# codebits1001/CET-driven-simulation-for-3D-printing-AM-KMC-Approach

Hardware: NVIDIA B200
Metric: kmc_site_updates_per_s (higher is better)
Workload: dtype f64

## Files before the change

cet-driven-simulation-for-3d-printing-am-kmc-approach_b200/csrc/rates_refresh.cu:

```cuda
#include <algorithm>
#include "ctx.cuh"
#include "pair_walk.cuh"
#include "tile_state.cuh"

namespace cet {

int rate_tables_ensure(cet_ctx *c);
int sm_count(cet_ctx *c);

constexpr int RF_THREADS = 256, RF_WARPS = RF_THREADS / 32;
enum { RF_KM_EMPTY = 1u << 8, RF_KP_EMPTY = 1u << 9, RF_K_GT0 = 1u << 10, RF_K_LTL = 1u << 11 };

template <int ROWS>
struct RefreshSmem {
    static constexpr int RF_CHUNK = RF_WARPS * ROWS * 32;
    double op[RF_WARPS][14][32];
    double tab[RT_TABLE_DOUBLES];
    uint64_t lw[RF_CHUNK];
    int32_t ls[RF_CHUNK];
    uint32_t lc[RF_CHUNK];
    int n_list[2][2];
    unsigned int chunk[2];
};

struct RefreshArgs {
    const uint8_t *cvox;
    const double *pairop, *T;
    double *site_rate, *dep_rate;
    const double *tab;
    const int32_t *list;
    const unsigned int *n_list;
    unsigned int *queue;
    cet_rate_params P;
    int L, n0, i_off;
    int top_lo, top_hi;
    unsigned int mLL, mL;
    int lin[14];
};

__device__ __forceinline__ int fast_div(int n, int d, unsigned int m, int *rem)
{
    int q = (int)__umulhi((unsigned int)n, m);
    int r = n - q * d;
    if (r < 0) { --q; r += d; }
    *rem = r;
    return q;
}
__device__ __forceinline__ void cp_async8(uint32_t dst, const void *src)
{
    asm volatile("cp.async.ca.shared.global [%0], [%1], 8;" ::"r"(dst), "l"(src) : "memory");
}
__device__ __forceinline__ void cp_async_wait_all()
{
    asm volatile("cp.async.commit_group;\ncp.async.wait_group 0;" ::: "memory");
}

template <bool ATT>
__device__ __noinline__ double rf_pairs_slow(const cet_rate_params &P, const double *tab, int cnt, uint32_t opaddr, double A, double B, double sum)
{
    for (int r = 0; r < cnt; ++r) {
        const double op = lds_f64(opaddr + 256u * (uint32_t)r);
        sum += ATT ? att_pair_rate_E(P, op, A, B, tab) : diff_pair_rate(P, A, B, op);
    }
    return sum;
}
template <bool ATT>
__device__ __forceinline__ double rf_pairs(const cet_rate_params &P, const double *exp_tab, int cnt, uint32_t opaddr, double A, double B,
                                           const double sum0)
{
    double sum = sum0;
    int xmax = 0;
    uint32_t addr = opaddr;
    for (int r = 0; r < cnt; r += 2, addr += 512u) {
        const bool two = r + 1 < cnt;
        const double op0 = lds_f64(addr);
        double op1 = 0.0;
        if (two) op1 = lds_f64(addr + 256u);
        const double r0 = pair_rate_raw<ATT>(P, exp_tab, op0, A, B, xmax);
        const double r1 = pair_rate_raw<ATT>(P, exp_tab, op1, A, B, xmax);
        add_kept(P, sum, r0);
        if (two) add_kept(P, sum, r1);
    }
    if (ATT && xmax >= EXP_RANGE_HI) sum = rf_pairs_slow<ATT>(P, exp_tab, cnt, opaddr, A, B, sum0);
    return sum;
}

template <int ROWS>
__global__ void __launch_bounds__(RF_THREADS, 4) rates_refresh_kernel(const __grid_constant__ RefreshArgs a)
{
    constexpr int RF_CHUNK = RF_WARPS * ROWS * 32, RF_ROWS = ROWS;
    extern __shared__ __align__(16) unsigned char refresh_dyn_smem[];
    RefreshSmem<ROWS> &sm = *reinterpret_cast<RefreshSmem<ROWS> *>(refresh_dyn_smem);
    const cet_rate_params &P = a.P;
    const int tid = threadIdx.x, lane = tid & 31, wid = tid >> 5;
    const int L = a.L, LL = L * L;
    const unsigned lt_mask = (1u << lane) - 1u;
    const int n = (int)*a.n_list;

    for (int q = tid; q < RT_TABLE_DOUBLES; q += RF_THREADS) sm.tab[q] = a.tab[q];
    if (tid == 0) {
        sm.chunk[0] = atomicAdd(a.queue, 1u);
        sm.n_list[0][0] = 0; sm.n_list[0][1] = 0;
    }
    __syncthreads();
    const uint32_t op0 = (uint32_t)__cvta_generic_to_shared(&sm.op[wid][0][lane]);

    for (unsigned it = 0;; ++it) {
        const int64_t c0 = (int64_t)sm.chunk[it & 1u] * RF_CHUNK;
        if (c0 >= n) break;
        int *n_list = sm.n_list[it & 1u];
        if (tid == 0) {
            sm.chunk[(it + 1u) & 1u] = atomicAdd(a.queue, 1u);
            sm.n_list[(it + 1u) & 1u][0] = 0; sm.n_list[(it + 1u) & 1u][1] = 0;
        }
        const int hi = (int)(c0 + RF_CHUNK < n ? c0 + RF_CHUNK : n);

#pragma unroll
        for (int r = 0; r < RF_ROWS; ++r) {
            const int q = (int)c0 + 32 * (wid * RF_ROWS + r) + lane;
            const bool active = q < hi;
            const int s = active ? a.list[q] : 0;
            int rem, k;
            const int p = fast_div(s, LL, a.mLL, &rem), j = fast_div(rem, L, a.mL, &k);
            const int gi = a.i_off + p;
            const bool interior = (unsigned)(gi - 2) < (unsigned)(a.n0 - 4) && (unsigned)(j - 2) < (unsigned)(L - 4) &&
                                  (unsigned)(k - 2) < (unsigned)(L - 4);
            unsigned inb = 0x3FFFu;
            if (!__all_sync(0xffffffffu, interior || !active)) inb = inbounds_mask(gi, j, k, a.n0, L);
            const uint8_t *cs = a.cvox + s;
            unsigned c = 0, b[14], km = 0, kp = 0;
#pragma unroll
            for (int o = 0; o < 14; ++o) b[o] = 0;
            if (active) {
                c = cs[0];
                if (k > 0) km = cs[-1];
                if (k < L - 1) kp = cs[1];
#pragma unroll
                for (int o = 0; o < 14; ++o)
                    if (inb >> o & 1u) b[o] = cs[a.lin[o]];
            }
            uint32_t wlo = 0, whi = 0;
#pragma unroll
            for (int o = 0; o < 8; ++o) wlo += (b[o] & 15u) << (4 * o);
#pragma unroll
            for (int o = 8; o < 14; ++o) whi += (b[o] & 15u) << (4 * (o - 8));
            const unsigned code = c & 15u;
            const bool is_emp = active && code == TC_EMPTY;
            const bool is_occ = active && (code & 1u) && code != TC_DEFECT;
            const uint32_t emp = (~wlo & (wlo >> 3) & 0x11111111u) | (~whi & (whi >> 3) & 0x00111111u);
            const bool to_att = is_emp, to_diff = is_occ && emp != 0u;
            if (active && !to_att && !to_diff) {
                a.site_rate[s] = 0.0;
                if (s >= a.top_lo && s < a.top_hi) a.dep_rate[s - a.top_lo] = NAN;
            }
            const unsigned b_att = __ballot_sync(0xffffffffu, to_att), b_diff = __ballot_sync(0xffffffffu, to_diff);
            if (b_att | b_diff) {
                int base_a = 0, base_d = 0;
                if (lane == 0) {
                    if (b_att) base_a = atomicAdd(&n_list[0], __popc(b_att));
                    if (b_diff) base_d = atomicAdd(&n_list[1], __popc(b_diff));
                }
                base_a = __shfl_sync(0xffffffffu, base_a, 0); base_d = __shfl_sync(0xffffffffu, base_d, 0);
                const uint32_t ent = c | ((km & 15u) == TC_EMPTY ? RF_KM_EMPTY : 0u) | ((kp & 15u) == TC_EMPTY ? RF_KP_EMPTY : 0u) |
                                     (k > 0 ? RF_K_GT0 : 0u) | (k < L - 1 ? RF_K_LTL : 0u);
                const uint64_t w = (uint64_t)wlo | ((uint64_t)whi << 32);
                int pos = -1;
                if (to_att) pos = base_a + __popc(b_att & lt_mask);
                if (to_diff) pos = RF_CHUNK - 1 - base_d - __popc(b_diff & lt_mask);
                if (pos >= 0) { sm.lw[pos] = w; sm.ls[pos] = s; sm.lc[pos] = ent; }
            }
        }
        __syncthreads();

        const int n_att = n_list[0], n_diff = n_list[1];
        const int nb_att = (n_att + 31) >> 5, nb_all = nb_att + ((n_diff + 31) >> 5);
#pragma unroll 1
        for (int bt = wid; bt < nb_all; bt += RF_WARPS) {
            const bool att = bt < nb_att;
            const int q = att ? 32 * bt + lane : 32 * (bt - nb_att) + lane;
            const bool on = q < (att ? n_att : n_diff);
            const int pos = att ? q : RF_CHUNK - 1 - q;
            uint64_t w = 0;
            uint32_t e = 0;
            int s = 0;
            if (on) { w = sm.lw[pos]; s = sm.ls[pos]; e = sm.lc[pos]; }
            const uint64_t pm = !on ? 0ull : att ? (w & (w >> 3) & CET_NIB_LSB) : (~w & (w >> 3) & CET_NIB_LSB);
            const uint32_t pm_lo = (uint32_t)pm, pm_hi = (uint32_t)(pm >> 32);
            const int cnt = __popc(pm_lo) + __popc(pm_hi);
            {
                const double *src = a.pairop + s;
                uint32_t dst = op0;
#pragma unroll
                for (int o = 0; o < 14; ++o) {
                    if ((o < 8 ? pm_lo >> (4 * o) : pm_hi >> (4 * (o - 8))) & 1u) {
                        cp_async8(dst, src + a.lin[o]);
                        dst += 256u;
                    }
                }
            }
            if (att) {
                double T_self = 1.0, T_m = 1.0, T_p = 1.0;
                if (on) {
                    T_self = a.pairop[s];
                    T_m = T_self; T_p = T_self;
                    if (pm) {
                        if (e & RF_K_GT0) T_m = (e & RF_KM_EMPTY) ? a.pairop[s - 1] : a.T[s - 1];
                        if (e & RF_K_LTL) T_p = (e & RF_KP_EMPTY) ? a.pairop[s + 1] : a.T[s + 1];
                    }
                }
                const TilePrep pr = tile_prep_emp(P, sm.tab, w, T_self, T_m, T_p);
                cp_async_wait_all();
                if (on) {
                    a.site_rate[s] = cnt ? rf_pairs<true>(P, sm.tab + RT_EXP2, cnt, op0, pr.A, pr.B, pr.sum0) : pr.sum0;
                    if (s >= a.top_lo && s < a.top_hi) {
                        double dep;
                        a.dep_rate[s - a.top_lo] = dep_rate(P, T_self, &dep) ? dep : NAN;
                    }
                }
            } else {
                const double T_self = on ? a.T[s] : 1.0;
                const unsigned c = e & 255u;
                const TilePrep pr = tile_prep_occ(P, sm.tab, w, c & 15u, (int)(c >> 4), T_self);
                cp_async_wait_all();
                if (on) {
                    a.site_rate[s] = rf_pairs<false>(P, sm.tab + RT_EXP2, cnt, op0, pr.A, pr.B, 0.0);
                    if (s >= a.top_lo && s < a.top_hi) a.dep_rate[s - a.top_lo] = NAN;
                }
            }
        }
        __syncthreads();
    }
}

template <int ROWS>
static int refresh_launch(cet_ctx *c, const RefreshArgs &a, int64_t nsite_hint, int *blocks_per_sm)
{
    constexpr int CHUNK = RF_WARPS * ROWS * 32;
    const size_t smem = sizeof(RefreshSmem<ROWS>);
    if (*blocks_per_sm == 0) {
        CET_CUDA(cudaFuncSetAttribute(rates_refresh_kernel<ROWS>, cudaFuncAttributeMaxDynamicSharedMemorySize, (int)smem));
        int nb = 0;
        CET_CUDA(cudaOccupancyMaxActiveBlocksPerMultiprocessor(&nb, rates_refresh_kernel<ROWS>, RF_THREADS, smem));
        CET_REQUIRE(nb >= 1, "rates_refresh_kernel does not fit an SM");
        *blocks_per_sm = nb;
    }
    const int grid = (int)std::min<int64_t>((nsite_hint + CHUNK - 1) / CHUNK, (int64_t)sm_count(c) * *blocks_per_sm);
    rates_refresh_kernel<ROWS><<<grid, RF_THREADS, smem, c->stream>>>(a);
    CET_CUDA(cudaGetLastError());
    return 0;
}

int rates_refresh_list(cet_ctx *c, const int32_t *list, const unsigned int *counter, int64_t nsite_hint)
{
    if (int rc = rate_tables_ensure(c)) return rc;
    RefreshArgs a;
    memset(&a, 0, sizeof(a));
    a.cvox = c->cvox; a.pairop = c->pairop; a.T = c->T;
    a.site_rate = c->site_rate; a.dep_rate = c->dep_rate; a.tab = c->rate_tab;
    a.list = list; a.n_list = counter;
    a.queue = (unsigned int *)(c->rate_tab + RT_TABLE_DOUBLES) + 3;
    a.P = c->rp;
    a.L = (int)c->n1; a.n0 = (int)c->n0; a.i_off = (int)(c->i_begin - c->halo);
    const int64_t top = c->n0 - 1 - (c->i_begin - c->halo);
    if (top >= 0 && top < c->np) { a.top_lo = (int)(top * c->plane); a.top_hi = (int)((top + 1) * c->plane); }
    a.mLL = (unsigned int)((1ull << 32) / (uint64_t)c->plane) + 1u;
    a.mL = (unsigned int)((1ull << 32) / (uint64_t)c->n1) + 1u;
    for (int o = 0; o < 14; ++o) a.lin[o] = (h_nb_off[o][0] * a.L + h_nb_off[o][1]) * a.L + h_nb_off[o][2];
    CET_CUDA(cudaMemsetAsync(a.queue, 0, sizeof(unsigned int), c->stream));
    const int v = (c->debug_flags & 1048576) ? 0 : (c->debug_flags & 2097152) ? 2 : 1;
    if (v == 0) return refresh_launch<1>(c, a, nsite_hint, &c->refresh_blocks[0]);
    if (v == 2) return refresh_launch<4>(c, a, nsite_hint, &c->refresh_blocks[2]);
    return refresh_launch<2>(c, a, nsite_hint, &c->refresh_blocks[1]);
}

}
```

Baseline: 99.30 billion.

## Pipeline rate refresh: classify next chunk while computing current, sort by neighbor-count key

Restructures the refresh kernel so each thread classifies one site of the next chunk while the block computes rates for the current chunk. cp.async prefetch of pair operands and temperatures is issued during the classify phase rather than inside the compute loop. Listed sites are bucketed by class and pair count with match_any and a warp scan, so each warp handles sites with similar loop trip counts and less divergence. Results are staged in shared memory and written back coalesced by the owning thread. The cost is more shared memory, extra syncs per chunk, and a more complex chunk queue with two chunks in flight.

```diff
diff --git a/cet-driven-simulation-for-3d-printing-am-kmc-approach_b200/csrc/rates_refresh.cu b/cet-driven-simulation-for-3d-printing-am-kmc-approach_b200/csrc/rates_refresh.cu
--- a/cet-driven-simulation-for-3d-printing-am-kmc-approach_b200/csrc/rates_refresh.cu
+++ b/cet-driven-simulation-for-3d-printing-am-kmc-approach_b200/csrc/rates_refresh.cu
@@ -8,18 +8,21 @@
 int rate_tables_ensure(cet_ctx *c);
 int sm_count(cet_ctx *c);
 
-constexpr int RF_THREADS = 256, RF_WARPS = RF_THREADS / 32;
-enum { RF_KM_EMPTY = 1u << 8, RF_KP_EMPTY = 1u << 9, RF_K_GT0 = 1u << 10, RF_K_LTL = 1u << 11 };
-
-template <int ROWS>
+enum : uint32_t {
+    RF_KM_EMPTY = 1u << 8, RF_KP_EMPTY = 1u << 9, RF_K_GT0 = 1u << 10, RF_K_LTL = 1u << 11,
+    RF_LISTED = 1u << 12, RF_TOP = 1u << 13, RF_KEY_SHIFT = 14, RF_RANK_SHIFT = 19
+};
+constexpr uint64_t RF_CODES = 0x00FFFFFFFFFFFFFFull;
+
+template <int THREADS>
 struct RefreshSmem {
-    static constexpr int RF_CHUNK = RF_WARPS * ROWS * 32;
-    double op[RF_WARPS][14][32];
+    static constexpr int CHUNK = THREADS;
+    double op[14][CHUNK];
+    double sT[3][CHUNK];
+    uint64_t sw[CHUNK];
     double tab[RT_TABLE_DOUBLES];
-    uint64_t lw[RF_CHUNK];
-    int32_t ls[RF_CHUNK];
-    uint32_t lc[RF_CHUNK];
-    int n_list[2][2];
+    int key_cnt[2][32], key_start[2][32];
+    int n_cls[2][2];
     unsigned int chunk[2];
 };
 
@@ -55,197 +58,250 @@
     asm volatile("cp.async.commit_group;\ncp.async.wait_group 0;" ::: "memory");
 }
 
-template <bool ATT>
+template <bool ATT, uint32_t STRIDE>
 __device__ __noinline__ double rf_pairs_slow(const cet_rate_params &P, const double *tab, int cnt, uint32_t opaddr, double A, double B, double sum)
 {
     for (int r = 0; r < cnt; ++r) {
-        const double op = lds_f64(opaddr + 256u * (uint32_t)r);
+        const double op = lds_f64(opaddr + STRIDE * (uint32_t)r);
         sum += ATT ? att_pair_rate_E(P, op, A, B, tab) : diff_pair_rate(P, A, B, op);
     }
     return sum;
 }
-template <bool ATT>
+template <bool ATT, uint32_t STRIDE>
 __device__ __forceinline__ double rf_pairs(const cet_rate_params &P, const double *exp_tab, int cnt, uint32_t opaddr, double A, double B,
                                            const double sum0)
 {
     double sum = sum0;
     int xmax = 0;
     uint32_t addr = opaddr;
-    for (int r = 0; r < cnt; r += 2, addr += 512u) {
+    for (int r = 0; r < cnt; r += 2, addr += 2u * STRIDE) {
         const bool two = r + 1 < cnt;
         const double op0 = lds_f64(addr);
         double op1 = 0.0;
-        if (two) op1 = lds_f64(addr + 256u);
+        if (two) op1 = lds_f64(addr + STRIDE);
         const double r0 = pair_rate_raw<ATT>(P, exp_tab, op0, A, B, xmax);
         const double r1 = pair_rate_raw<ATT>(P, exp_tab, op1, A, B, xmax);
         add_kept(P, sum, r0);
         if (two) add_kept(P, sum, r1);
     }
-    if (ATT && xmax >= EXP_RANGE_HI) sum = rf_pairs_slow<ATT>(P, exp_tab, cnt, opaddr, A, B, sum0);
+    if (ATT && xmax >= EXP_RANGE_HI) sum = rf_pairs_slow<ATT, STRIDE>(P, exp_tab, cnt, opaddr, A, B, sum0);
     return sum;
 }
 
-template <int ROWS>
-__global__ void __launch_bounds__(RF_THREADS, 4) rates_refresh_kernel(const __grid_constant__ RefreshArgs a)
-{
-    constexpr int RF_CHUNK = RF_WARPS * ROWS * 32, RF_ROWS = ROWS;
+template <int THREADS>
+__global__ void __launch_bounds__(THREADS, 1024 / THREADS) rates_refresh_kernel(const __grid_constant__ RefreshArgs a)
+{
+    using Smem = RefreshSmem<THREADS>;
+    constexpr int CHUNK = Smem::CHUNK, WARPS = THREADS / 32;
+    constexpr uint32_t STRIDE = 8u * CHUNK;
     extern __shared__ __align__(16) unsigned char refresh_dyn_smem[];
-    RefreshSmem<ROWS> &sm = *reinterpret_cast<RefreshSmem<ROWS> *>(refresh_dyn_smem);
+    Smem &sm = *reinterpret_cast<Smem *>(refresh_dyn_smem);
     const cet_rate_params &P = a.P;
     const int tid = threadIdx.x, lane = tid & 31, wid = tid >> 5;
     const int L = a.L, LL = L * L;
     const unsigned lt_mask = (1u << lane) - 1u;
     const int n = (int)*a.n_list;
-
-    for (int q = tid; q < RT_TABLE_DOUBLES; q += RF_THREADS) sm.tab[q] = a.tab[q];
-    if (tid == 0) {
-        sm.chunk[0] = atomicAdd(a.queue, 1u);
-        sm.n_list[0][0] = 0; sm.n_list[0][1] = 0;
-    }
+    const uint32_t op0 = (uint32_t)__cvta_generic_to_shared(&sm.op[0][0]);
+    const uint32_t sT0 = (uint32_t)__cvta_generic_to_shared(&sm.sT[0][0]);
+    const unsigned past_end = (unsigned)(n / CHUNK + 1);
+    auto chunk_start = [&](unsigned e) { return (int)min(e, past_end) * CHUNK; };
+
+    auto classify = [&](int s_in, int b, uint64_t &w, uint32_t &lc) {
+        const bool active = s_in >= 0;
+        const int s = active ? s_in : 0;
+        int rem, k;
+        const int p = fast_div(s, LL, a.mLL, &rem), j = fast_div(rem, L, a.mL, &k);
+        const int gi = a.i_off + p;
+        const bool interior = (unsigned)(gi - 2) < (unsigned)(a.n0 - 4) && (unsigned)(j - 2) < (unsigned)(L - 4) &&
+                              (unsigned)(k - 2) < (unsigned)(L - 4);
+        unsigned inb = 0x3FFFu;
+        if (!__all_sync(0xffffffffu, interior || !active)) inb = inbounds_mask(gi, j, k, a.n0, L);
+        const uint8_t *cs = a.cvox + s;
+        unsigned c = 0, bc[14], km = 0, kp = 0;
+#pragma unroll
+        for (int o = 0; o < 14; ++o) bc[o] = 0;
+        if (active) {
+            c = cs[0];
+            if (k > 0) km = cs[-1];
+            if (k < L - 1) kp = cs[1];
+#pragma unroll
+            for (int o = 0; o < 14; ++o)
+                if (inb >> o & 1u) bc[o] = cs[a.lin[o]];
+        }
+        uint32_t wlo = 0, whi = 0;
+#pragma unroll
+        for (int o = 0; o < 8; ++o) wlo += (bc[o] & 15u) << (4 * o);
+#pragma unroll
+        for (int o = 8; o < 14; ++o) whi += (bc[o] & 15u) << (4 * (o - 8));
+        const unsigned code = c & 15u;
+        const bool is_emp = active && code == TC_EMPTY;
+        const bool is_occ = active && (code & 1u) && code != TC_DEFECT;
+        const uint32_t att = (wlo & (wlo >> 3) & 0x11111111u) | (whi & (whi >> 3) & 0x00111111u);
+        const uint32_t emp = (~wlo & (wlo >> 3) & 0x11111111u) | (~whi & (whi >> 3) & 0x00111111u);
+        const bool to_att = is_emp, to_diff = is_occ && emp != 0u;
+        const bool listed = to_att || to_diff;
+        const int key = (to_att ? 0 : 16) + __popc(to_att ? att : emp);
+        const unsigned peers = __match_any_sync(0xffffffffu, listed ? key : -1);
+        int rank = 0;
+        if (listed) {
+            const int leader = __ffs(peers) - 1;
+            if (lane == leader) rank = atomicAdd(&sm.key_cnt[b][key], __popc(peers));
+            rank = __shfl_sync(peers, rank, leader) + __popc(peers & lt_mask);
+        }
+        lc = (active && s >= a.top_lo && s < a.top_hi) ? RF_TOP : 0u;
+        if (listed)
+            lc |= c | ((km & 15u) == TC_EMPTY ? RF_KM_EMPTY : 0u) | ((kp & 15u) == TC_EMPTY ? RF_KP_EMPTY : 0u) | (k > 0 ? RF_K_GT0 : 0u) |
+                  (k < L - 1 ? RF_K_LTL : 0u) | RF_LISTED | ((uint32_t)key << RF_KEY_SHIFT) | ((uint32_t)rank << RF_RANK_SHIFT);
+        w = (uint64_t)wlo | ((uint64_t)whi << 32);
+    };
+    auto scan_keys = [&](int b) {
+        const int cnt = sm.key_cnt[b][lane];
+        int inc = cnt;
+#pragma unroll
+        for (int d = 1; d < 32; d <<= 1) {
+            const int u = __shfl_up_sync(0xffffffffu, inc, d);
+            if (lane >= d) inc += u;
+        }
+        const int n_emp = __shfl_sync(0xffffffffu, inc, 15);
+        sm.key_start[b][lane] = inc - cnt - (lane >= 16 ? n_emp : 0);
+        sm.key_cnt[b][lane] = 0;
+        if (lane == 31) { sm.n_cls[b][0] = n_emp; sm.n_cls[b][1] = inc - n_emp; }
+    };
+    auto sorted_pos = [&](uint32_t lc, int b) {
+        const int key = (int)((lc >> RF_KEY_SHIFT) & 31u);
+        const int i = sm.key_start[b][key] + (int)(lc >> RF_RANK_SHIFT);
+        return key < 16 ? i : CHUNK - 1 - i;
+    };
+
+    for (int q = tid; q < RT_TABLE_DOUBLES; q += THREADS) sm.tab[q] = a.tab[q];
+    if (tid < 64) sm.key_cnt[tid >> 5][tid & 31] = 0;
+    if (tid == 0) { sm.chunk[0] = atomicAdd(a.queue, 1u); sm.chunk[1] = atomicAdd(a.queue, 1u); }
     __syncthreads();
-    const uint32_t op0 = (uint32_t)__cvta_generic_to_shared(&sm.op[wid][0][lane]);
-
-    for (unsigned it = 0;; ++it) {
-        const int64_t c0 = (int64_t)sm.chunk[it & 1u] * RF_CHUNK;
-        if (c0 >= n) break;
-        int *n_list = sm.n_list[it & 1u];
-        if (tid == 0) {
-            sm.chunk[(it + 1u) & 1u] = atomicAdd(a.queue, 1u);
-            sm.n_list[(it + 1u) & 1u][0] = 0; sm.n_list[(it + 1u) & 1u][1] = 0;
-        }
-        const int hi = (int)(c0 + RF_CHUNK < n ? c0 + RF_CHUNK : n);
-
-#pragma unroll
-        for (int r = 0; r < RF_ROWS; ++r) {
-            const int q = (int)c0 + 32 * (wid * RF_ROWS + r) + lane;
-            const bool active = q < hi;
-            const int s = active ? a.list[q] : 0;
-            int rem, k;
-            const int p = fast_div(s, LL, a.mLL, &rem), j = fast_div(rem, L, a.mL, &k);
-            const int gi = a.i_off + p;
-            const bool interior = (unsigned)(gi - 2) < (unsigned)(a.n0 - 4) && (unsigned)(j - 2) < (unsigned)(L - 4) &&
-                                  (unsigned)(k - 2) < (unsigned)(L - 4);
-            unsigned inb = 0x3FFFu;
-            if (!__all_sync(0xffffffffu, interior || !active)) inb = inbounds_mask(gi, j, k, a.n0, L);
-            const uint8_t *cs = a.cvox + s;
-            unsigned c = 0, b[14], km = 0, kp = 0;
-#pragma unroll
-            for (int o = 0; o < 14; ++o) b[o] = 0;
-            if (active) {
-                c = cs[0];
-                if (k > 0) km = cs[-1];
-                if (k < L - 1) kp = cs[1];
-#pragma unroll
-                for (int o = 0; o < 14; ++o)
-                    if (inb >> o & 1u) b[o] = cs[a.lin[o]];
+    int c_cur = chunk_start(sm.chunk[0]);
+    int s_cur = c_cur + tid < n ? a.list[c_cur + tid] : -1, s_nxt = -1, s_pre;
+    uint64_t w_cur = 0, w_nxt = 0;
+    uint32_t lc_cur = 0, lc_nxt = 0;
+    if (c_cur < n) classify(s_cur, 0, w_cur, lc_cur);
+    {
+        const int c = chunk_start(sm.chunk[1]);
+        s_pre = c + tid < n ? a.list[c + tid] : -1;
+    }
+    __syncthreads();
+    if (wid == 0) scan_keys(0);
+    __syncthreads();
+
+    for (unsigned it = 0; c_cur < n; ++it) {
+        const int cur = it & 1u, nxt = cur ^ 1;
+        const int c_nxt = chunk_start(sm.chunk[nxt]);
+
+        if (lc_cur & RF_LISTED) {
+            const int pos = sorted_pos(lc_cur, cur);
+            const bool att = ((lc_cur >> RF_KEY_SHIFT) & 31u) < 16u;
+            const uint64_t w = w_cur, pm = att ? (w & (w >> 3) & CET_NIB_LSB) : (~w & (w >> 3) & CET_NIB_LSB);
+            const int s = s_cur;
+            const uint32_t pm_lo = (uint32_t)pm, pm_hi = (uint32_t)(pm >> 32);
+            const double *src = a.pairop + s;
+            uint32_t dst = op0 + 8u * (uint32_t)pos;
+#pragma unroll
+            for (int o = 0; o < 14; ++o) {
+                if ((o < 8 ? pm_lo >> (4 * o) : pm_hi >> (4 * (o - 8))) & 1u) {
+                    cp_async8(dst, src + a.lin[o]);
+                    dst += STRIDE;
+                }
             }
-            uint32_t wlo = 0, whi = 0;
-#pragma unroll
-            for (int o = 0; o < 8; ++o) wlo += (b[o] & 15u) << (4 * o);
-#pragma unroll
-            for (int o = 8; o < 14; ++o) whi += (b[o] & 15u) << (4 * (o - 8));
-            const unsigned code = c & 15u;
-            const bool is_emp = active && code == TC_EMPTY;
-            const bool is_occ = active && (code & 1u) && code != TC_DEFECT;
-            const uint32_t emp = (~wlo & (wlo >> 3) & 0x11111111u) | (~whi & (whi >> 3) & 0x00111111u);
-            const bool to_att = is_emp, to_diff = is_occ && emp != 0u;
-            if (active && !to_att && !to_diff) {
-                a.site_rate[s] = 0.0;
-                if (s >= a.top_lo && s < a.top_hi) a.dep_rate[s - a.top_lo] = NAN;
+            const uint32_t tdst = sT0 + 8u * (uint32_t)pos;
+            uint64_t fl;
+            if (att) {
+                cp_async8(tdst, a.pairop + s);
+                if (pm) {
+                    if (lc_cur & RF_K_GT0) cp_async8(tdst + STRIDE, ((lc_cur & RF_KM_EMPTY) ? a.pairop : a.T) + (s - 1));
+                    if (lc_cur & RF_K_LTL) cp_async8(tdst + 2u * STRIDE, ((lc_cur & RF_KP_EMPTY) ? a.pairop : a.T) + (s + 1));
+                }
+                fl = ((lc_cur >> 10) & 3u) | ((lc_cur & RF_TOP) ? 4u : 0u);
+            } else {
+                cp_async8(tdst, a.T + s);
+                fl = lc_cur & 255u;
             }
-            const unsigned b_att = __ballot_sync(0xffffffffu, to_att), b_diff = __ballot_sync(0xffffffffu, to_diff);
-            if (b_att | b_diff) {
-                int base_a = 0, base_d = 0;
-                if (lane == 0) {
-                    if (b_att) base_a = atomicAdd(&n_list[0], __popc(b_att));
-                    if (b_diff) base_d = atomicAdd(&n_list[1], __popc(b_diff));
-                }
-                base_a = __shfl_sync(0xffffffffu, base_a, 0); base_d = __shfl_sync(0xffffffffu, base_d, 0);
-                const uint32_t ent = c | ((km & 15u) == TC_EMPTY ? RF_KM_EMPTY : 0u) | ((kp & 15u) == TC_EMPTY ? RF_KP_EMPTY : 0u) |
-                                     (k > 0 ? RF_K_GT0 : 0u) | (k < L - 1 ? RF_K_LTL : 0u);
-                const uint64_t w = (uint64_t)wlo | ((uint64_t)whi << 32);
-                int pos = -1;
-                if (to_att) pos = base_a + __popc(b_att & lt_mask);
-                if (to_diff) pos = RF_CHUNK - 1 - base_d - __popc(b_diff & lt_mask);
-                if (pos >= 0) { sm.lw[pos] = w; sm.ls[pos] = s; sm.lc[pos] = ent; }
-            }
-        }
+            sm.sw[pos] = w | (fl << 56);
+        }
+        if (c_nxt < n) {
+            s_nxt = s_pre;
+            classify(s_nxt, nxt, w_nxt, lc_nxt);
+        }
+        cp_async_wait_all();
         __syncthreads();
-
-        const int n_att = n_list[0], n_diff = n_list[1];
+        if (tid == 0) sm.chunk[cur] = atomicAdd(a.queue, 1u);
+        if (wid == 0 && c_nxt < n) scan_keys(nxt);
+
+        const int n_att = sm.n_cls[cur][0], n_diff = sm.n_cls[cur][1];
         const int nb_att = (n_att + 31) >> 5, nb_all = nb_att + ((n_diff + 31) >> 5);
 #pragma unroll 1
-        for (int bt = wid; bt < nb_all; bt += RF_WARPS) {
+        for (int bt = wid; bt < nb_all; bt += WARPS) {
             const bool att = bt < nb_att;
             const int q = att ? 32 * bt + lane : 32 * (bt - nb_att) + lane;
             const bool on = q < (att ? n_att : n_diff);
-            const int pos = att ? q : RF_CHUNK - 1 - q;
+            const int pos = att ? q : CHUNK - 1 - q;
             uint64_t w = 0;
-            uint32_t e = 0;
-            int s = 0;
-            if (on) { w = sm.lw[pos]; s = sm.ls[pos]; e = sm.lc[pos]; }
-            const uint64_t pm = !on ? 0ull : att ? (w & (w >> 3) & CET_NIB_LSB) : (~w & (w >> 3) & CET_NIB_LSB);
-            const uint32_t pm_lo = (uint32_t)pm, pm_hi = (uint32_t)(pm >> 32);
-            const int cnt = __popc(pm_lo) + __popc(pm_hi);
-            {
-                const double *src = a.pairop + s;
-                uint32_t dst = op0;
-#pragma unroll
-                for (int o = 0; o < 14; ++o) {
-                    if ((o < 8 ? pm_lo >> (4 * o) : pm_hi >> (4 * (o - 8))) & 1u) {
-                        cp_async8(dst, src + a.lin[o]);
-                        dst += 256u;
-                    }
-                }
-            }
+            double T_self = 1.0;
+            if (on) { w = sm.sw[pos]; T_self = sm.sT[0][pos]; }
+            const unsigned fl = (unsigned)(w >> 56);
+            w &= RF_CODES;
+            const uint32_t opaddr = op0 + 8u * (uint32_t)pos;
             if (att) {
-                double T_self = 1.0, T_m = 1.0, T_p = 1.0;
-                if (on) {
-                    T_self = a.pairop[s];
-                    T_m = T_self; T_p = T_self;
-                    if (pm) {
-                        if (e & RF_K_GT0) T_m = (e & RF_KM_EMPTY) ? a.pairop[s - 1] : a.T[s - 1];
-                        if (e & RF_K_LTL) T_p = (e & RF_KP_EMPTY) ? a.pairop[s + 1] : a.T[s + 1];
-                    }
+                const uint64_t pm = w & (w >> 3) & CET_NIB_LSB;
+                double T_m = T_self, T_p = T_self;
+                if (pm) {
+                    if (fl & 1u) T_m = sm.sT[1][pos];
+                    if (fl & 2u) T_p = sm.sT[2][pos];
                 }
                 const TilePrep pr = tile_prep_emp(P, sm.tab, w, T_self, T_m, T_p);
-                cp_async_wait_all();
+                const int cnt = popc64(pm);
                 if (on) {
-                    a.site_rate[s] = cnt ? rf_pairs<true>(P, sm.tab + RT_EXP2, cnt, op0, pr.A, pr.B, pr.sum0) : pr.sum0;
-                    if (s >= a.top_lo && s < a.top_hi) {
+                    sm.sT[0][pos] = cnt ? rf_pairs<true, STRIDE>(P, sm.tab + RT_EXP2, cnt, opaddr, pr.A, pr.B, pr.sum0) : pr.sum0;
+                    if (fl & 4u) {
                         double dep;
-                        a.dep_rate[s - a.top_lo] = dep_rate(P, T_self, &dep) ? dep : NAN;
+                        sm.sT[1][pos] = dep_rate(P, T_self, &dep) ? dep : NAN;
                     }
                 }
             } else {
-                const double T_self = on ? a.T[s] : 1.0;
-                const unsigned c = e & 255u;
-                const TilePrep pr = tile_prep_occ(P, sm.tab, w, c & 15u, (int)(c >> 4), T_self);
-                cp_async_wait_all();
-                if (on) {
-                    a.site_rate[s] = rf_pairs<false>(P, sm.tab + RT_EXP2, cnt, op0, pr.A, pr.B, 0.0);
-                    if (s >= a.top_lo && s < a.top_hi) a.dep_rate[s - a.top_lo] = NAN;
-                }
+                const TilePrep pr = tile_prep_occ(P, sm.tab, w, fl & 15u, (int)(fl >> 4), T_self);
+                if (on) sm.sT[0][pos] = rf_pairs<false, STRIDE>(P, sm.tab + RT_EXP2, popc64(pr.pm), opaddr, pr.A, pr.B, 0.0);
             }
         }
         __syncthreads();
-    }
-}
-
-template <int ROWS>
+
+        if (s_cur >= 0) {
+            const bool listed = lc_cur & RF_LISTED;
+            const int pos = listed ? sorted_pos(lc_cur, cur) : 0;
+            a.site_rate[s_cur] = listed ? sm.sT[0][pos] : 0.0;
+            if (lc_cur & RF_TOP) {
+                const bool emp = listed && ((lc_cur >> RF_KEY_SHIFT) & 31u) < 16u;
+                a.dep_rate[s_cur - a.top_lo] = emp ? sm.sT[1][pos] : NAN;
+            }
+        }
+        {
+            const int c = chunk_start(sm.chunk[cur]);
+            s_pre = c + tid < n ? a.list[c + tid] : -1;
+        }
+        c_cur = c_nxt; s_cur = c_nxt < n ? s_nxt : -1; w_cur = w_nxt; lc_cur = lc_nxt;
+        __syncthreads();
+    }
+}
+
+template <int THREADS>
 static int refresh_launch(cet_ctx *c, const RefreshArgs &a, int64_t nsite_hint, int *blocks_per_sm)
 {
-    constexpr int CHUNK = RF_WARPS * ROWS * 32;
-    const size_t smem = sizeof(RefreshSmem<ROWS>);
+    constexpr int CHUNK = RefreshSmem<THREADS>::CHUNK;
+    const size_t smem = sizeof(RefreshSmem<THREADS>);
     if (*blocks_per_sm == 0) {
-        CET_CUDA(cudaFuncSetAttribute(rates_refresh_kernel<ROWS>, cudaFuncAttributeMaxDynamicSharedMemorySize, (int)smem));
+        CET_CUDA(cudaFuncSetAttribute(rates_refresh_kernel<THREADS>, cudaFuncAttributeMaxDynamicSharedMemorySize, (int)smem));
         int nb = 0;
-        CET_CUDA(cudaOccupancyMaxActiveBlocksPerMultiprocessor(&nb, rates_refresh_kernel<ROWS>, RF_THREADS, smem));
+        CET_CUDA(cudaOccupancyMaxActiveBlocksPerMultiprocessor(&nb, rates_refresh_kernel<THREADS>, THREADS, smem));
         CET_REQUIRE(nb >= 1, "rates_refresh_kernel does not fit an SM");
         *blocks_per_sm = nb;
     }
     const int grid = (int)std::min<int64_t>((nsite_hint + CHUNK - 1) / CHUNK, (int64_t)sm_count(c) * *blocks_per_sm);
-    rates_refresh_kernel<ROWS><<<grid, RF_THREADS, smem, c->stream>>>(a);
+    rates_refresh_kernel<THREADS><<<grid, THREADS, smem, c->stream>>>(a);
     CET_CUDA(cudaGetLastError());
     return 0;
 }
@@ -267,10 +323,9 @@
     a.mL = (unsigned int)((1ull << 32) / (uint64_t)c->n1) + 1u;
     for (int o = 0; o < 14; ++o) a.lin[o] = (h_nb_off[o][0] * a.L + h_nb_off[o][1]) * a.L + h_nb_off[o][2];
     CET_CUDA(cudaMemsetAsync(a.queue, 0, sizeof(unsigned int), c->stream));
-    const int v = (c->debug_flags & 1048576) ? 0 : (c->debug_flags & 2097152) ? 2 : 1;
-    if (v == 0) return refresh_launch<1>(c, a, nsite_hint, &c->refresh_blocks[0]);
-    if (v == 2) return refresh_launch<4>(c, a, nsite_hint, &c->refresh_blocks[2]);
-    return refresh_launch<2>(c, a, nsite_hint, &c->refresh_blocks[1]);
-}
-
-}
+    if (c->debug_flags & 1048576) return refresh_launch<128>(c, a, nsite_hint, &c->refresh_blocks[0]);
+    if (c->debug_flags & 2097152) return refresh_launch<512>(c, a, nsite_hint, &c->refresh_blocks[2]);
+    return refresh_launch<256>(c, a, nsite_hint, &c->refresh_blocks[1]);
+}
+
+}
```

Result: no change. 100.3 billion, median of 6 (+1.0%).
